# tuffy/libdvd-audio

Measured on AMD Instinct MI355X. Metric: decoded PCM Msamples/s (bit-exact) on 6ch/96k/24b MLP, higher is better.
Workload: dtype int32 (int64 accumulate)

## Files before the change

libdvd-audio_amd/csrc/mlp_decode.h:

```cpp
#pragma once
#include <hip/hip_runtime.h>
#if defined(__HIP_DEVICE_COMPILE__) && !defined(__gfx950__)
#error "mlp_decode.h is written for gfx950 (MI355X): hand-placed s_waitcnt encodings and gfx950 inline asm"
#endif
#include <stdint.h>
#include <type_traits>
#include "mlp_bounds.h"
#include "mlp_index.h"
#include "mlp_tables.h"

namespace mlp {

constexpr int DEC_THREADS = 128;
constexpr int DEC_WAVES = DEC_THREADS / 64;
constexpr int MAXCH = 8;
constexpr int MAXMAT = 6;
constexpr int RING_PLANES = 8;
constexpr int RING_DWORDS = RING_PLANES * 4;
constexpr int CHUNK_DWORDS = 16;
constexpr int OUT_ROWS = 4;
constexpr uint32_t YIELD_LONELY = 48;
#ifndef DVDA_HDR_GATE_TURNS
#define DVDA_HDR_GATE_TURNS 32
#endif
// ... 133 lines not shown
    uint32_t total_lanes;
    unsigned long long *dbg;
    int32_t *fir_ws;
    int32_t *fb;
    const int32_t *init_fir;
    DecodeSummary *summary;
    uint32_t interleaved;
    uint32_t wav_bits;
    uint32_t coop_min_seg;
    const uint32_t *hetero;
    const uint32_t *lane_seg;
    const uint32_t *cls;
    uint32_t only_S;
    uint32_t *seg_meta;
    uint32_t *yield_req;
    const uint32_t *seg_check;
    const uint32_t *list;
    uint32_t list_base, list_n;
    const uint32_t *list_n_ptr;
    const uint4 *plan;
    int32_t *res;
    uint32_t *brec;
    uint32_t *frec;
    WsCaps caps;
    uint32_t coop;
    struct CoopState *coop_state;
    struct CoopResult *coop_result;
    uint32_t coop_fresh;
};

constexpr uint32_t COOP_MAX_SEG = 4096;
constexpr uint32_t COOP_MAX_AU = 32768;
__device__ __forceinline__ bool coop_takes(const DecodeArgs &a)
{
    if (a.coop)
        return a.coop == 64u;
    uint32_t n_seg = *a.n_seg_ptr;
    if (n_seg > a.max_seg)
        n_seg = a.max_seg;
    return n_seg <= COOP_MAX_SEG && a.seg_fbase[n_seg] <= COOP_MAX_AU;
}



__device__ __forceinline__ int32_t mask_q(int32_t x, uint32_t q)
{
    return (int32_t)((uint32_t)x & (0xFFFFFFFFu << q));
}
__device__ __forceinline__ uint32_t nib(uint32_t pack, uint32_t i) { return (pack >> (4 * i)) & 0xFu; }
__device__ __forceinline__ int32_t lo16(uint32_t v) { return (int32_t)(v << 16) >> 16; }
__device__ __forceinline__ int32_t hi16(uint32_t v) { return (int32_t)v >> 16; }

__device__ __forceinline__ int32_t huff_center(uint32_t codebook, uint32_t lb)
{
    if (codebook) {
        const int ss = (int)lb + 2 - (int)codebook;
        return 7 * (1 << lb) + (ss >= 0 ? (1 << ss) : 0);
    }
    const int ss = (int)lb - 1;
    return ss >= 0 ? (1 << ss) : 0;
}

__device__ __forceinline__ uint32_t be32(uint32_t v) { return __builtin_bswap32(v); }
template <int RD = RING_DWORDS>
__device__ __forceinline__ void ring_store16(uint32_t *dst, const uint4 &a, const uint4 &b, const uint4 &c,
                                             const uint4 &d, bool first_plane)
{
    const uint32_t a0 = be32(a.x);
    uint32_t *const e = dst - 15 * 64;
    if (first_plane)
        dst[-RD * 64] = a0;
    e[15 * 64] = a0;         e[14 * 64] = be32(a.y); e[13 * 64] = be32(a.z); e[12 * 64] = be32(a.w);
    e[11 * 64] = be32(b.x);  e[10 * 64] = be32(b.y); e[9 * 64] = be32(b.z);  e[8 * 64] = be32(b.w);
    e[7 * 64] = be32(c.x);   e[6 * 64] = be32(c.y);  e[5 * 64] = be32(c.z);  e[4 * 64] = be32(c.w);
    e[3 * 64] = be32(d.x);   e[2 * 64] = be32(d.y);  e[1 * 64] = be32(d.z);  e[0 * 64] = be32(d.w);
}

template <int RD>
__device__ __forceinline__ void ring_store4(uint32_t *dst, const uint4 &a, bool first_plane)
{
    const uint32_t a0 = be32(a.x);
    if (first_plane)
        dst[-RD * 64] = a0;
    dst[0] = a0;
    dst[-1 * 64] = be32(a.y);
    dst[-2 * 64] = be32(a.z);
    dst[-3 * 64] = be32(a.w);
}

__device__ __forceinline__ void ring_fill_sync(const uint4 *src, uint32_t *dst, bool first_plane)
{
    const uint4 a = src[0], b = src[1], c = src[2], d = src[3];
    ring_store16(dst, a, b, c, d, first_plane);
}

__device__ __attribute__((noinline)) int64_t iir_mac(const int32_t *ws, uint32_t stride)
{
    int64_t acc = 0;
    for (uint32_t j = 0; j < 8; j++)
        acc += (int64_t)ws[(size_t)j * stride] * (int64_t)ws[(size_t)(8 + j) * stride];
    return acc;
}

__device__ __attribute__((noinline)) void iir_push(int32_t *ws, uint32_t stride, int32_t v)
{
    for (int j = 7; j > 0; j--)
        ws[(size_t)(8 + j) * stride] = ws[(size_t)(8 + j - 1) * stride];
    ws[(size_t)8 * stride] = v;
}

template <int RD, int G>
struct BitReaderT {
    const uint4 *gsrc;
    uint32_t *ring;
    uint32_t max_chunk;
    uint32_t pos;
    uint32_t fillpos;
    uint32_t lo_valid;

    __device__ __forceinline__ uint32_t *slot(uint32_t d) const
    {
        return ring + ((RD - (d & (RD - 1))) << 6);
    }
    __device__ __forceinline__ uint64_t window() const
    {
        const uint32_t *p = ring + ((~(pos >> 5) & (RD - 1)) << 6);
        return ((uint64_t)p[64] << 32) | p[0];
    }
    __device__ __forceinline__ uint32_t window_lds() const
    {
        return (uint32_t)(uintptr_t)ring + ((~(pos >> 5) & (RD - 1)) << 8);
    }
    __device__ __forceinline__ int32_t ahead() const
    {
        return (int32_t)((fillpos << 5) - (pos & ~31u)) >> 5;
    }
    __device__ __forceinline__ void filled()
    {
        fillpos += G;
        if (fillpos - lo_valid > (uint32_t)RD)
            lo_valid = fillpos - RD;
    }
    __device__ __forceinline__ uint32_t fill_src() const
    {
        const uint32_t last = max_chunk + (uint32_t)(CHUNK_DWORDS - G);
        return fillpos < last ? fillpos : last;
    }
    __device__ __forceinline__ bool room() const { return ahead() <= (int32_t)(RD - G); }
    __device__ __forceinline__ void fill_sync()
    {
        if constexpr (G == CHUNK_DWORDS) {
            ring_fill_sync(gsrc + (fill_src() >> 2), slot(fillpos), (fillpos & (RD - 1)) == 0);
            filled();
        } else {
            uint4 q[4];
            const int32_t n = fill_issue(q);
            fill_commit(q, n);
        }
    }
    template <int MAXG = 4>
    __device__ __forceinline__ int32_t fill_issue(uint4 (&q)[MAXG]) const
    {
        static_assert(G == CHUNK_DWORDS || (G == 4 && RD == 16), "the small ring is 16 dwords filled by 16-byte granules");
        int32_t n = room() ? (RD - ahead()) >> 2 : 0;
        if (MAXG < 4 && n > MAXG)
            n = MAXG;
#pragma unroll
        for (int g = 0; g < MAXG; g++)
            if (g < n) {
                const uint32_t f = fillpos + 4u * g, last = max_chunk + (uint32_t)(CHUNK_DWORDS - G);
                q[g] = gsrc[(f < last ? f : last) >> 2];
            }
        return n;
    }
    template <int MAXG = 4>
    __device__ __forceinline__ void fill_commit(const uint4 (&q)[MAXG], int32_t n)
    {
#pragma unroll
        for (int g = 0; g < MAXG; g++)
            if (g < n) {
                ring_store4<RD>(slot(fillpos), q[g], (fillpos & (RD - 1)) == 0);
                filled();
            }
    }
    __device__ __forceinline__ void ensure(uint32_t n)
    {
#if defined(DVDA_EXP_STAMP)
        const unsigned long long t0_ = clock64();
        bool any_ = false;
#endif
        while (__builtin_expect(__any(ahead() < (int32_t)n), 0)) {
            if (room())
                fill_sync();
#if defined(DVDA_EXP_STAMP)
            any_ = true;
#endif
        }
#if defined(DVDA_EXP_STAMP)
        if (any_) {
            fill_cyc += clock64() - t0_;
            fill_n++;
        }
#endif
    }
#if defined(DVDA_EXP_STAMP)
    unsigned long long fill_cyc = 0, fill_n = 0;
#endif
    __device__ __forceinline__ void seek_byte(uint64_t byte_pos)
    {
        const uint32_t t = (uint32_t)(byte_pos >> 2);
        if (!((int32_t)(t - lo_valid) >= 0 && (int32_t)(fillpos - t) > 0)) {
            fillpos = t & ~(uint32_t)(G - 1);
            lo_valid = fillpos;
        }
        pos = (uint32_t)byte_pos << 3;
    }
    __device__ __forceinline__ uint64_t tell_near(uint64_t ref_bits) const
    {
        return ref_bits + (uint64_t)(int64_t)(int32_t)(pos - (uint32_t)ref_bits);
    }
    __device__ __forceinline__ bool past(uint32_t end_bits_lo) const { return (int32_t)(pos - end_bits_lo) > 0; }
    __device__ __forceinline__ uint32_t peek32()
    {
        ensure(2);
        return (uint32_t)((window() << (pos & 31u)) >> 32);
    }
    __device__ __forceinline__ uint32_t read(uint32_t n)
    {
        const uint32_t top = peek32();
        pos += n;
        return n ? top >> (32 - n) : 0u;
    }
    __device__ __forceinline__ uint32_t read_resident(uint32_t n)
    {
        const uint32_t top = (uint32_t)((window() << (pos & 31u)) >> 32);
        pos += n;
        return (top >> 1) >> (31u - n);
    }
    __device__ __forceinline__ int32_t read_signed_resident(uint32_t n)
    {
        const uint32_t top = (uint32_t)((window() << (pos & 31u)) >> 32);
        pos += n;
        return n ? (int32_t)top >> ((32u - n) & 31u) : 0;
    }
    __device__ __forceinline__ int32_t read_signed(uint32_t n)
    {
        if (n == 0)
            return 0;
        const int32_t v = (int32_t)peek32() >> (32 - n);
        pos += n;
        return v;
    }
};

using BitReader = BitReaderT<RING_DWORDS, CHUNK_DWORDS>;
constexpr int DUO_RING = 16, DUO_GRAN = 4;

__host__ __device__ constexpr uint32_t hot_word(uint32_t cb, uint32_t lb, uint32_t q, uint32_t shift)
{
    return lb | (q << 5) | ((shift + q) << 10) |
           (cb ? ((7u - (8u >> cb)) << 16) | ((cb == 1 ? 9u : cb == 2 ? 7u : 6u) << 20) | ((4u - cb) << 24) |
                 ((28u + cb) << 26) | (1u << 31)
               : 0u);
}
__device__ __forceinline__ uint32_t hot_cb(uint32_t hw) { return (hw >> 26) & 3u; }
__device__ __forceinline__ uint32_t hot_lb(uint32_t hw) { return hw & 31u; }
__device__ __forceinline__ uint32_t hot_q(uint32_t hw) { return (hw >> 5) & 15u; }
__host__ __device__ constexpr uint32_t cold_word(uint32_t iir_order, uint32_t fir_order, uint32_t fir_shift, uint32_t iir_shift)
{
    return iir_order | (fir_order << 4) | (fir_shift << 8) | (iir_shift << 12);
}

__device__ __forceinline__ uint32_t huff_decode_top(uint32_t top, uint32_t hw)
{
    const uint32_t a = (top >> ((hw >> 26) & 31u)) + ((hw >> 16) & 0x307u);
    const uint32_t n = (uint32_t)__clz((int)((top & 0x3F800000u) | 0x00400000u));
    const uint32_t up = ((hw >> 20) & 0x10Fu) + n, dn = 0x108u - n;
    uint32_t d = 0x40000000u - (top & 0x7F800000u);
    asm("" : "+v"(d));
    uint32_t ms = (uint32_t)((int32_t)d >> 31);
    asm("" : "+v"(ms));
    uint32_t val = (up & ms) | (dn & ~ms);
    asm("" : "+v"(val));
    const uint32_t e = (n << 8) + val;
    uint32_t m = (uint32_t)((int32_t)top >> 31);
    asm("" : "+v"(m));
    return ((a & m) | (e & ~m)) & (uint32_t)((int32_t)hw >> 31);
}

__device__ __forceinline__ uint32_t huff_decode(uint32_t cb, uint32_t t)
{
    return huff_decode_top(t << 23, hot_word(cb, 0u, 0u, 0u));
}

struct SubPark {
    uint32_t flags, block_size, min_ch, max_ch, max_mat_ch, noise_shift, seed, matrix_len, bypass_mask, outch_pack,
             oshift_pack, qss_pack, nslots, iir_any, ss_end_bit, rows_left, blocks_in_frame, chk, gl, seg_lane;
    bool have_restart, seg_iir;
    uint32_t *brec, *brec_end, *brec_base;
};

template <int NS, bool PAIRED, bool GENERAL, bool ILV = false, bool PARSE = false, bool DUO = false, bool WAVO = false>
__global__ __launch_bounds__(DEC_THREADS, 2) void k_decode(DecodeArgs a)
{
    static_assert(!(GENERAL && PARSE), "one mode at a time");
    static_assert(!DUO || (!PAIRED && !GENERAL && NS == 6), "the two-substream lane is a one-lane fast-pass / parse instance");
    static_assert(GENERAL == PAIRED, "lane pairs are the sequential pass's layout, and its only one");
    constexpr uint32_t L = PAIRED ? 2u : 1u;
    if (!GENERAL && a.only_S && a.cls[a.only_S - 1u] == 0)
        return;
    if (!GENERAL && !PARSE && coop_takes(a))
        return;
    constexpr int THREADS = DEC_THREADS;
    constexpr int WAVES = THREADS / 64;
    constexpr int TP = 6;
    constexpr int RD = DUO ? DUO_RING : RING_DWORDS;
    constexpr int RG = DUO ? DUO_GRAN : CHUNK_DWORDS;
    using Reader = BitReaderT<RD, RG>;
    __shared__ uint32_t s_ring[WAVES][DUO ? 2 : 1][RD + 1][64];
    __shared__ int32_t s_out[GENERAL ? 1 : WAVES][TP][OUT_ROWS][GENERAL ? 1 : 64];
    constexpr bool XCH = PAIRED;
    __shared__ int32_t s_xch[XCH ? WAVES : 1][MAXCH][XCH ? 64 : 1];
    __shared__ uint32_t s_nchained[WAVES];
    __shared__ uint16_t s_cold[WAVES][NS][64];

    if (threadIdx.x < WAVES)
        s_nchained[threadIdx.x] = 0;
    __syncthreads();

    const int lane = threadIdx.x & 63;
    const int wv = threadIdx.x >> 6;
    const uint32_t wg_id = blockIdx.x;
    const uint32_t gl0 = wg_id * THREADS + threadIdx.x;
    uint32_t n_seg = *a.n_seg_ptr;
    if (n_seg > a.max_seg)
        n_seg = a.max_seg;
    const uint32_t item = gl0 / L;
    uint32_t segi = item;
    bool active = segi < n_seg;
    if (!GENERAL && !PARSE && active && *a.hetero)
        segi = DVDA_AT(a.lane_seg, item, a.caps.max_seg, BT_LANE_SEG);
    if (!GENERAL && !PARSE && segi >= n_seg) {
        active = false;
        segi = n_seg;
    }
    if (GENERAL || PARSE) {
        active = item < a.list_n && (a.list_n_ptr == nullptr || item < *a.list_n_ptr) && (!PARSE || item < DVDA_AT(a.plan, n_seg, a.caps.max_seg + 1u, BT_PLAN).y);
        segi = 0;
        if (active) {
            const uint32_t e = DVDA_AT(a.list, a.list_base + item, GENERAL ? a.caps.max_streams : a.caps.max_seg, BT_LIST);
            segi = GENERAL ? DVDA_AT(a.streams, e, a.caps.max_streams, BT_STREAMS).first_seg : e;
            active = segi < n_seg;
        }
        if (!active)
            segi = n_seg;
    }

    SegRec sr;
    sr.off = sr.end = 0;
    sr.stream = 0;
    sr.nframes = 0;
    sr.flags = 0;
    sr.sync = 0;
    sr.ndrop = 0;
    sr.prev = 0xFFFFFFFFu;
    uint32_t fbase = 0, stream_sync = 0, stream_first = 0;
    if (active) {
        sr = DVDA_AT(a.seg, segi, a.caps.max_seg, BT_SEG);
        stream_first = DVDA_AT(a.streams, sr.stream, a.caps.max_streams, BT_STREAMS).first_seg;
        if (stream_first == 0xFFFFFFFFu) {
            active = false;
            stream_first = segi;
        } else {
            stream_sync = a.streams[sr.stream].sync;
            fbase = a.seg_fbase[segi] - DVDA_AT(a.seg_fbase, stream_first, a.caps.max_seg + 1u, BT_FBASE);
        }
    }
    const uint32_t S = (stream_sync >> 24) & 0xF;
    const uint32_t sub = DUO ? 1u : gl0 - item * L;
    uint32_t gl = segi * 2u + sub;
    uint32_t seg_lane = gl;
    const uint32_t assignment = (stream_sync >> 16) & 0x1F;
    const uint32_t rpa = rows_per_au((stream_sync >> 8) & 0xF);
    const uint32_t nch_out = channel_count(assignment);
    const uint32_t wavepk = wave_pack(assignment);
    const uint32_t wave_inv = ILV ? wave_inv_pack(assignment) : 0u;
    uint32_t status = 0;
    if (active && (sr.flags & ST_FATAL_INDEX))
        active = false;
    if (active && (sub >= S || sr.nframes == 0))
        active = false;
    bool mine = GENERAL || !a.only_S || S == a.only_S;
    if (!mine)
        active = false;
    if (active && S > (DUO ? 2u : L)) {
        status |= ST_ENVELOPE;
        active = false;
    }
    if (DUO && S != 2u)
        active = false;
    if (active && (rpa == 0 || nch_out == 0)) {
        status |= ST_ENVELOPE;
        active = false;
    }
    const bool is_last_sub = (sub + 1 == S);
    const bool owner = is_last_sub;

    uint64_t out_base = 0, out_stride = 0;
    if (active && !PARSE) {
        out_base = a.out_off[sr.stream];
        out_stride = a.out_stride[sr.stream];
    }
    uint64_t row0 = (uint64_t)fbase * rpa;
    uint64_t row_limit = row0 + (uint64_t)(sr.nframes - sr.ndrop) * rpa;
    constexpr bool seq = GENERAL;
    bool resume_from_init = false;
    int32_t *fbuf = nullptr;
    if (GENERAL && active) {
        const uint32_t st_j = a.seg_status[segi];
        if (st_j & ST_CHAINED) {
            if (a.init_fir)
                resume_from_init = true;
            else {
                status |= ST_ENVELOPE;
                active = false;
            }
        }
        fbuf = a.fb + (size_t)item * FB_WORDS;
        if (active && !DVDA_RANGE_OK((size_t)item * FB_WORDS, FB_WORDS, a.caps.fb, BT_FB)) {
            status |= ST_CAPACITY;
            active = false;
        }
        if (active) {
            atomicAnd(&a.seg_status[segi], ST_DEFERRED | ST_FATAL_INDEX | ST_TRUNCATED | ST_SYNC_CHANGE);
            row0 = 0;
            row_limit = ~0ull;
        }
    }
    uint32_t seg_R = 0;
    uint32_t *brec = nullptr, *brec_end = nullptr, *brec_base = nullptr;
    uint32_t *frec = nullptr;
    if (PARSE && active) {
        const uint4 pl = DVDA_AT(a.plan, segi, a.caps.max_seg + 1u, BT_PLAN);
        const uint32_t st_j = a.seg_status[segi];
        seg_R = (sr.nframes - sr.ndrop) * rpa;
        out_base = (uint64_t)pl.x * 8u;
        out_stride = seg_R;
        row0 = 0;
        row_limit = seg_R;
        const uint32_t cap = brec_capacity(seg_R);
        brec = a.brec + brec_offset(pl.x, pl.y, sub, seg_R);
        brec_base = brec;
        brec_end = brec + cap;
        frec = a.frec + (uint64_t)(pl.x / 40u) * FREC_WORDS;
        (void)st_j;
        atomicAnd(&a.seg_status[segi], ST_DEFERRED | ST_FATAL_INDEX | ST_TRUNCATED | ST_SYNC_CHANGE);
        if (!DVDA_RANGE_OK(out_base, 8ull * seg_R, a.caps.res, BT_RES) ||
            !DVDA_RANGE_OK(brec_offset(pl.x, pl.y, sub, seg_R), cap, a.caps.brec, BT_BREC) ||
            !DVDA_RANGE_OK((uint64_t)(pl.x / 40u) * FREC_WORDS, (uint64_t)(sr.nframes - sr.ndrop) * FREC_WORDS, a.caps.frec, BT_FREC)) {
            status |= ST_CAPACITY;
            active = false;
        }
    }
    if (active && !DVDA_RANGE_OK(gl, 1, a.caps.lanes, BT_META)) {
        status |= ST_CAPACITY;
        active = false;
    }
    uint32_t room = 0;
    {
        const uint64_t edge = out_stride < row_limit ? out_stride : row_limit;
// ... 723 lines not shown
                                    }
                                    if (fir_order && frames_done == 0 && blocks_in_frame == 0)
                                        status |= ST_CHAINED;
                                    const int32_t nsho = hoff - huff_center(codebook, lb);
                                    const uint32_t npk = hot_word(codebook, lb, q, shift);
                                    if (kr < (uint32_t)NS)
                                        *cold = (uint16_t)cold_word(iir_order, fir_order, fir_shift, iir_shift);
#pragma unroll
                                    for (int kk = 0; kk < NS; kk++)
                                        if ((uint32_t)kk == kr) {
                                            pk[kk] = npk;
                                            sho[kk] = nsho;
                                            if (new_fir) {
#pragma unroll
                                                for (int j = 0; j < 4; j++) {
                                                    if constexpr (!CFU) {
                                                        cf[kk][CFU ? 0 : j] = (int32_t)ncf[j];
                                                    } else {
                                                        cf[kk][CFU ? 2 * j : 0] = lo16(ncf[j]);
                                                        cf[kk][CFU ? 2 * j + 1 : 0] = hi16(ncf[j]);
                                                    }
                                                }
                                            }
                                        }
                                    iir_any = (iir_any & ~(1u << k)) | ((iir_order ? 1u : 0u) << k);
                                    if (PARSE) {
                                        const bool with_iir = new_iir && iir_order != 0;
                                        if (brec + 2 * BREC_STRIDE + (with_iir ? BREC_IIR_WORDS : 0) > brec_end) {
                                            seq_needed = true;
                                        } else {
                                            uint32_t *w = brec + BREC_SLOT * k;
                                            w[2] = shift | (q << 4) | (fir_order << 8) | (iir_order << 12) |
                                                   (new_iir ? 1u << 16 : 0u);
#pragma unroll
                                            for (int j = 0; j < 4; j++)
                                                w[3 + j] = new_fir ? ncf[j] : cf_old[j];
                                            w[7] = 0;
                                            chg_mask |= 1u << k;
                                            if (with_iir) {
                                                const int32_t *ws = a.iir_ws + (size_t)(k * 16) * a.total_lanes + gl;
                                                brec_end -= BREC_IIR_WORDS;
                                                uint32_t *x = brec_end;
                                                for (uint32_t j = 0; j < 4; j++)
                                                    x[j] = ((uint32_t)ws[(size_t)(2 * j) * a.total_lanes] & 0xFFFFu) |
                                                           ((uint32_t)ws[(size_t)(2 * j + 1) * a.total_lanes] << 16);
                                                for (uint32_t j = 0; j < 8; j++)
                                                    x[4 + j] = (uint32_t)ws[(size_t)(8 + j) * a.total_lanes];
                                                w[7] = (uint32_t)(x - brec_base);
                                            }
                                        }
                                    }
                                }
                            }
                        }
                    }
                }
                DVDA_HSTAMP(3);
                if (!have_restart && ok) {
                    ok = false;
                    err = no_restart_yet();
                }
                hdr_parsed = true;
                if (PARSE && iir_any)
                    seg_iir = true;
                if (PARSE && ok && chg_mask) {
#pragma unroll
                    for (int kk = 0; kk < 6; kk++) {
                        brec[BREC_SLOT * kk] = rows_done;
                        brec[BREC_SLOT * kk + 1] = (chg_mask >> kk) & 1u;
                    }
                    brec += BREC_STRIDE;
                }
                if (PARSE && ok && (seq_needed || (hdr_restart && blocks_in_frame))) {
                    status |= ST_SEQ;
                    active = false;
                }
                if (mat_mine) {
                    qss_A = qss_pack;
                    mmc_A = max_mat_ch;
                }
                const uint32_t cold_ml = matrix_len;
                if (matrix_class_change)
                    status |= ST_MIDFRAME;
                if (!ok) {
                    status |= err;
                    active = false;
                } else if (PARSE && !active) {
                } else if (!GENERAL && !PARSE && (iir_any != 0 || cold_ml > 2)) {
                    status |= ST_COLD;
                    active = false;
                } else if (!GENERAL && !PARSE && (status & ST_CHAINED)) {
                    active = false;
                    if (!(DUO && probe))
                        atomicAdd(&s_nchained[wv], 1u);
                    if (sr.prev != 0xFFFFFFFFu)
                        __hip_atomic_store(&DVDA_AT(a.yield_req, sr.prev, a.caps.max_seg, BT_YIELD), 1u, __ATOMIC_RELAXED, __HIP_MEMORY_SCOPE_AGENT);
                } else {
                    rows_left = block_size;
                    blocks_in_frame++;
                    if (!GENERAL && !PARSE && frames_done < 2 &&
                        __hip_atomic_load(&s_nchained[wv], __ATOMIC_RELAXED, __HIP_MEMORY_SCOPE_WORKGROUP) >= YIELD_LONELY) {
                        status |= ST_YIELD;
                        active = false;
                    }
                }
            }
                if constexpr (DUO) {
                    if (pass == 0u && me)
                        swap_sub();
                    if (!PARSE && pass == 0u && me && !active && first0 && !(status & ~ST_INFO)) {
                        probe = true;
                        active = true;
                    }
                    if (pass == 1u && probe)
                        active = false;
                }
            }
            if constexpr (DUO) {
                if (active && have_restart && P0.have_restart && (P0.min_ch != 0u || min_ch != P0.max_ch + 1u)) {
                    status |= PARSE ? ST_SEQ : ST_COLD;
                    active = false;
                }
            }
        }
        if (hdr_now) {
            DVDA_HSTAMP(4);
#if defined(DVDA_EXP_STAMP)
            hstamp_acc[5] += rd.fill_cyc + (DUO ? rx.fill_cyc : 0ull);
            hfills += rd.fill_n + (DUO ? rx.fill_n : 0ull);
            hcount++;
#endif
        }
        if (!__any(active))
            break;
        DVDA_STAMP(0);

        if (active) {
            if constexpr (DUO) {
                while (__builtin_expect(__any(rd.ahead() < 8 || rx.ahead() < 8), 0)) {
                    DVDA_COV(14);
                    uint4 q[1];
                    const int32_t n0 = rx.template fill_issue<1>(q);
                    rx.template fill_commit<1>(q, n0);
                    const int32_t n1 = rd.template fill_issue<1>(q);
                    rd.template fill_commit<1>(q, n1);
                }
            } else {
            if (rd.ahead() < 12)
                DVDA_COV(14);
            rd.ensure(12);
            }
        }
        DVDA_STAMP(7);
        const bool pf = active && rd.room();
        const bool pfx = DUO && active && rx.room();
        uint4 p0, p1, p2, p3;
        asm volatile("" : "=v"(p0.x), "=v"(p0.y), "=v"(p0.z), "=v"(p0.w), "=v"(p1.x), "=v"(p1.y), "=v"(p1.z), "=v"(p1.w),
                          "=v"(p2.x), "=v"(p2.y), "=v"(p2.z), "=v"(p2.w), "=v"(p3.x), "=v"(p3.y), "=v"(p3.z), "=v"(p3.w));
        bool flush = false;
        const uint32_t frames_before = frames_done;
        uint64_t flush_row = 0;
        if constexpr (DUO) {
            if (pfx)
                p0 = rx.gsrc[rx.fill_src() >> 2];
            if (pf)
                p1 = rd.gsrc[rd.fill_src() >> 2];
        } else {
        if (pf) {
            const uint32_t c = rd.fillpos < rd.max_chunk ? rd.fillpos : rd.max_chunk;
            const uint4 *src = rd.gsrc + (c >> 2);
            p0 = src[0];
            p1 = src[1];
            p2 = src[2];
            p3 = src[3];
        }
        }
        DVDA_STAMP(1);

        uint32_t bypass_bits = 0;
        int32_t val[NS];
        auto row_head_any = [&]() {
            if (__any(bypass_mask != 0)) {
                const uint32_t cnt = (uint32_t)__popc(bypass_mask);
                const uint32_t field = rd.read_resident(cnt);
                const uint32_t b0 = bypass_mask & 1u, b1 = (bypass_mask >> 1) & 1u;
                bypass_bits = (b0 & (field >> ((cnt - 1u) & 31u))) | ((b1 & (field >> ((cnt - 1u - b0) & 31u))) << 1);
                if ((GENERAL || PARSE) && __builtin_expect(__any((bypass_mask >> 2) != 0), 0)) {
                    if (bypass_mask >> 2)
                        DVDA_COV(10);
                    uint32_t rank = b0 + b1;
#pragma unroll
                    for (int m = 2; m < MAXMAT; m++) {
                        const uint32_t bit = (bypass_mask >> m) & 1u;
                        bypass_bits |= (bit & (field >> ((cnt - 1u - rank) & 31u))) << m;
                        rank += bit;
                    }
                }
            }
            if constexpr (DUO)
                rx.pos += (uint32_t)__popc(P0.bypass_mask);
            uint32_t cpos = DUO ? rx.pos : rd.pos;
            uint32_t cbase = (uint32_t)(uintptr_t)(DUO ? rx.ring : rd.ring) + (uint32_t)((RD - 1) << 8);
            auto cur_window_lds = [&]() -> uint32_t { return cbase - ((cpos << 3) & (uint32_t)((RD - 1) << 8)); };
            uint64_t win = DUO ? rx.window() : rd.window();
            const uint32_t n_sub0 = DUO ? P0.max_ch + 1u : 0u;
            uint32_t msb_or = 0;
            const bool wave_iir = GENERAL && __any(iir_any != 0);
#pragma unroll
            for (int k = 0; k < NS; k++) {
                const bool in = DUO ? (uint32_t)k <= max_ch : (uint32_t)k < nslots;
                if (k > 0)
                    asm volatile("s_waitcnt lgkmcnt(0)" : "+v"(win));
                if constexpr (DUO) {
                    if (k > 0) {
                        const bool sw = (uint32_t)k == n_sub0;
                        if (__any(sw)) {
                            if (sw) {
                                rx.pos = cpos;
                                cpos = rd.pos;
                                cbase = (uint32_t)(uintptr_t)rd.ring + (uint32_t)((RD - 1) << 8);
                                win = rd.window();
                            }
                        }
                    }
                }
                val[k] = 0;
                if (k >= 2 && !__any(in))
                    continue;
                if (in) {
                const uint32_t hw = pk[k];
                const uint32_t lb = hw & 31u;
                const uint32_t ofs = cpos & 31u;
                const uint32_t top = (uint32_t)((win << ofs) >> 32);
                const uint32_t e = huff_decode_top(top, hw);
                const uint32_t msb = e & 0xFFu;
                const uint32_t len = e >> 8;
                msb_or |= msb;
                const uint32_t o2 = ofs + len;
                cpos += len + lb;
                const uint32_t top2 = (uint32_t)((win << o2) >> 32);
                const uint32_t lsbv = (top2 >> 1) >> (~hw & 31u);
                if (k + 1 < NS)
                    asm volatile("ds_read2st64_b32 %0, %2 offset1:1" : "+v"(win), "+v"(sp[k][0]) : "v"(cur_window_lds()));
                uint32_t ml = (msb << (hw & 31u)) + lsbv;
                asm("" : "+v"(ml));
                const uint32_t resq = ml + (uint32_t)sho[k];
                const uint32_t q5 = (hw >> 5) & 31u;
                int32_t value;
                if constexpr (PARSE) {
                    value = (int32_t)(resq << q5);
                    (void)wave_iir;
                } else {
                auto tap = [&](int j) -> int32_t {
                    if constexpr (CFU)
                        return cf[k][CFU ? j : 0];
                    else
                        return (j & 1) ? hi16((uint32_t)cf[k][CFU ? 0 : j >> 1]) : lo16((uint32_t)cf[k][CFU ? 0 : j >> 1]);
                };
                int64_t acc0 = (int64_t)tap(0) * (int64_t)st_get(k, 0);
                int64_t acc1 = (int64_t)tap(1) * (int64_t)st_get(k, 1);
                acc0 += (int64_t)tap(2) * (int64_t)st_get(k, 2);
                acc1 += (int64_t)tap(3) * (int64_t)st_get(k, 3);
                acc0 += (int64_t)tap(4) * (int64_t)st_get(k, 4);
                acc1 += (int64_t)tap(5) * (int64_t)st_get(k, 5);
                acc0 += (int64_t)tap(6) * (int64_t)st_get(k, 6);
                acc1 += (int64_t)tap(7) * (int64_t)st_get(k, 7);
                int64_t acc = acc0 + acc1;
                bool iir_on = false;
                if (__builtin_expect(wave_iir, 0)) {
                    iir_on = in && ((iir_any >> k) & 1u);
                    if (iir_on)
                        DVDA_COV(11);
                    if (iir_on)
                        acc += iir_mac(a.iir_ws + (size_t)(k * 16) * a.total_lanes + gl, a.total_lanes);
                }
                value = (int32_t)(((uint32_t)(acc >> ((hw >> 10) & 63u)) + resq) << q5);
                {
                    uint32_t vhi;
                    asm("" : "=v"(vhi));
                    const uint64_t vpair = (uint64_t)(uint32_t)value | ((uint64_t)vhi << 32);
                    asm("v_pk_mov_b32 %0, %1, %0 op_sel:[1,0]" : "+v"(sp[k][3]) : "v"(sp[k][2]));
                    asm("v_pk_mov_b32 %0, %1, %0 op_sel:[1,0]" : "+v"(sp[k][2]) : "v"(sp[k][1]));
                    asm("v_pk_mov_b32 %0, %1, %0 op_sel:[1,0]" : "+v"(sp[k][1]) : "v"(sp[k][0]));
                    asm("v_pk_mov_b32 %0, %1, %0 op_sel:[0,0]" : "+v"(sp[k][0]) : "v"(vpair));
                }
                if (__builtin_expect(wave_iir, 0)) {
                    if (iir_on) {
                        const int32_t ssum = (int32_t)(acc >> (((hw >> 10) & 63u) - hot_q(hw)));
                        iir_push(a.iir_ws + (size_t)(k * 16) * a.total_lanes + gl, a.total_lanes,
                                 (int32_t)((uint32_t)value - (uint32_t)ssum));
                    }
                }
                }
                val[k] = value;
                }
            }
            rd.pos = cpos;
            if (__builtin_expect((msb_or & 0x80u) != 0, 0)) {
                status |= ST_HUFFMAN;
                active = false;
            }
            DVDA_STAMP(2);
        };
        auto row_tail = [&](int32_t (&ch)[MAXCH]) {
            if (owner) {
                if (GENERAL) {
                    if (frame_rows >= (uint32_t)FB_ROWS) {
                        status |= ST_ENVELOPE;
                        active = false;
                    } else {
                        int32_t *fr = fbuf + (size_t)frame_rows * (MAXCH + 1);
#pragma unroll
                        for (int c = 0; c < MAXCH; c++)
                            fr[c] = ch[c];
                        fr[MAXCH] = (int32_t)bypass_bits;
                    }
                } else {
                    if constexpr (PARSE) {
#pragma unroll
// ... 85 lines not shown
                            uint32_t *F = frec + (size_t)au_idx * FREC_WORDS;
                            if (!DVDA_RANGE_OK((size_t)(F - a.frec), FREC_WORDS, a.caps.frec, BT_FREC))
                                F = a.frec;
                            F[0] = noise_shift | (matrix_len << 8) | (max_mat_ch << 16);
                            F[1] = outch_pack;
                            F[2] = qss_pack;
                            F[3] = oshift_pack;
#pragma unroll
                            for (int m = 0; m < 2; m++) {
#pragma unroll
                                for (int j = 0; j < 4; j++)
                                    F[4 + m * 5 + j] = mreg[m][j];
                                F[4 + m * 5 + 4] = mnoise[m];
                            }
                            for (uint32_t m = 2; m < matrix_len; m++)
                                for (uint32_t j = 0; j < 5; j++)
                                    F[4 + m * 5 + j] = a.mat_ws[(size_t)(m * 5 + j) * a.total_lanes + gl];
                        }
                        au_idx++;
                        in_frame = false;
                        frames_done++;
                    }
                }
            } else
            if (__builtin_expect(active && rows_left == 0, 0)) {
                if (rd.read(1)) {
                    if (frame_rows != rpa && !seq) {
                        status |= ST_TIMING;
                        active = false;
                    }
                    if (rd.past(ss_end_bit)) {
                        status |= ST_EOF;
                        active = false;
                    }
                    if (active && (chk >> 2) == frames_done) {
                        status |= (chk & 1u) ? ST_PARITY : ST_CRC;
                        active = false;
                    }
                    if (PARSE && is_last_sub && active) {
                        uint32_t *F = frec + (size_t)au_idx * FREC_WORDS;
                        if (!DVDA_RANGE_OK((size_t)(F - a.frec), FREC_WORDS, a.caps.frec, BT_FREC))
                            F = a.frec;
                        F[0] = noise_shift | (matrix_len << 8) | (max_mat_ch << 16);
                        F[1] = outch_pack;
                        F[2] = qss_pack;
                        F[3] = oshift_pack;
#pragma unroll
                        for (int m = 0; m < 2; m++) {
#pragma unroll
                            for (int j = 0; j < 4; j++)
                                F[4 + m * 5 + j] = mreg[m][j];
                            F[4 + m * 5 + 4] = mnoise[m];
                        }
                        for (uint32_t m = 2; m < matrix_len; m++)
                            for (uint32_t j = 0; j < 5; j++)
                                F[4 + m * 5 + j] = a.mat_ws[(size_t)(m * 5 + j) * a.total_lanes + gl];
                    }
                    au_idx++;
                    if (GENERAL && is_last_sub && active) {
                        const uint64_t frow0 = row - frame_rows;
                        for (uint32_t r = 0; r < frame_rows; r++) {
                            const int32_t *fr = fbuf + (size_t)r * (MAXCH + 1);
                            int32_t ch[MAXCH];
#pragma unroll
                            for (int c = 0; c < MAXCH; c++)
                                ch[c] = fr[c];
                            rematrix(ch, (uint32_t)fr[MAXCH]);
                            const uint64_t orow = frow0 + r;
                            if (orow >= out_stride) {
                                status |= ST_OVERFLOW;
                            } else {
                                if (a.wav_bits) {
                                    const uint32_t nb = a.wav_bits >> 3;
                                    uint8_t *wb = reinterpret_cast<uint8_t *>(a.pcm + out_base) + orow * nch_out * nb;
                                    for (uint32_t c = 0; c < nch_out && c < 6u; c++) {
                                        int32_t v = 0;
#pragma unroll
                                        for (int cc = 0; cc < 6; cc++)
                                            if ((uint32_t)cc == c)
                                                v = ch[cc];
                                        const uint32_t u = wav_signed(v, a.wav_bits);
                                        for (uint32_t b = 0; b < nb; b++)
                                            wb[nib(wavepk, c) * nb + b] = (uint8_t)(u >> (8 * b));
                                    }
                                } else {
#pragma unroll
                                for (int c = 0; c < 6; c++)
                                    if ((uint32_t)c < nch_out)
                                        a.pcm[out_base + (a.interleaved ? orow * nch_out + nib(wavepk, c)
                                                                        : (uint64_t)nib(wavepk, c) * out_stride + orow)] = ch[c];
                                }
                            }
                            rows_written++;
                        }
                    }
                    in_frame = false;
                    frames_done++;
                } else if (rd.past(ss_end_bit)) {
                    status |= ST_EOF;
                    active = false;
                }
            }
        };
        int32_t ch[MAXCH];
        const bool in_row = active && (!HDR_GATE || (rows_left != 0 && (!DUO || P0.rows_left != 0)));
        if (in_row) {
            row_head_any();
            if (PAIRED) {
                const int slot0 = lane & ~1;
                int32_t(*X)[XCH ? 64 : 1] = s_xch[XCH ? wv : 0];
#pragma unroll
                for (int k = 0; k < NS; k++)
                    if ((uint32_t)k < nslots && min_ch + k < MAXCH)
                        X[min_ch + k][XCH ? slot0 : 0] = val[k];
                __builtin_amdgcn_fence(__ATOMIC_RELEASE, "wavefront");
                __builtin_amdgcn_wave_barrier();
                __builtin_amdgcn_fence(__ATOMIC_ACQUIRE, "wavefront");
#pragma unroll
                for (int c = 0; c < MAXCH; c++)
                    ch[c] = X[c][XCH ? slot0 : 0];
            } else {
#pragma unroll
                for (int c = 0; c < MAXCH; c++)
                    ch[c] = c < NS ? val[c < NS ? c : 0] : 0;
            }
            row_tail(ch);
        }
        if constexpr (GENERAL) {
            const int ended = frames_done != frames_before ? 1 : 0;
            const int other = __shfl_xor(ended, 1, 64);
            if (S == 2u && active && ended != other) {
                status |= ST_ENVELOPE;
                active = false;
            }
        }
        DVDA_STAMP(3);

#if defined(DVDA_EXP_STAMP)
        {
            asm volatile("s_waitcnt vmcnt(0)" ::: "memory");
            DVDA_STAMP(6);
        }
#endif
        __builtin_amdgcn_s_waitcnt(0x0F70);
        if constexpr (DUO) {
            if (pfx) {
                ring_store4<RD>(rx.slot(rx.fillpos), p0, (rx.fillpos & (RD - 1)) == 0);
                rx.filled();
            }
            if (pf) {
                ring_store4<RD>(rd.slot(rd.fillpos), p1, (rd.fillpos & (RD - 1)) == 0);
                rd.filled();
            }
        } else {
        if (pf) {
            ring_store16(rd.slot(rd.fillpos), p0, p1, p2, p3, (rd.fillpos & (RING_DWORDS - 1)) == 0);
            rd.filled();
        }
        }
        bool coop_out = false;
        if constexpr (ILV && !GENERAL && !PARSE) {
            if (!WAVO && ilv_direct && a.wav_bits == 0u && a.coop_min_seg && n_seg >= a.coop_min_seg)
                coop_out = __ballot(flush) == ~0ull;
        }
        if (coop_out) {
            const uint64_t doff = out_base + flush_row * 6u;
            const bool off32 = !__any((doff >> 32) != 0);
            const uint32_t d_lo = (uint32_t)doff, d_hi = (uint32_t)(doff >> 32);
            const int32_t *const T0 = &s_out[GENERAL ? 0 : wv][0][0][0];
            const uint32_t l6 = ((uint32_t)lane * 43691u) >> 18;
            const uint32_t pc = (uint32_t)lane - l6 * 6u;
            const int32_t *const Tl6 = T0 + pc * (4 * 64) + l6;
            const bool l60 = lane < 60;
#pragma unroll
            for (uint32_t it7 = 0; it7 < 7u; it7++) {
                const uint32_t o = l6 + 10u * it7;
                const uint32_t b_lo = (uint32_t)__shfl((int)d_lo, (int)o, 64);
                uint64_t eo = b_lo;
                if (!off32)
                    eo |= (uint64_t)(uint32_t)__shfl((int)d_hi, (int)o, 64) << 32;
                if (l60 && (it7 < 6u || o < 64u)) {
                    int32_t *const od = a.pcm + eo + pc * 4u;
                    const int32_t *const Tp = Tl6 + 10u * it7;
                    DVDA_STORE_V4_COOP(od, Tp[0], Tp[64], Tp[128], Tp[192]);
                }
            }
        }
        if (!GENERAL && !PARSE && ILV && flush && !coop_out) {
            const int32_t *Tl = &s_out[GENERAL ? 0 : wv][0][0][GENERAL ? 0 : lane];
            int32_t *dst = a.pcm + out_base + flush_row * nch_out;
            constexpr bool WAV_ELSEWHERE = !PAIRED && !WAVO && !DUO;
            if (WAVO || (!WAV_ELSEWHERE && __builtin_expect(a.wav_bits != 0, 0))) {
                const uint32_t nb = a.wav_bits >> 3;
                uint32_t *wd = reinterpret_cast<uint32_t *>(a.pcm + out_base) + (flush_row * nch_out * nb >> 2);
                if (ilv_direct && a.wav_bits == 24u) {
                    uint32_t d[18];
#pragma unroll
                    for (int g = 0; g < 6; g++) {
                        const int32_t o[4] = {Tl[(4 * g) * 64], Tl[(4 * g + 1) * 64], Tl[(4 * g + 2) * 64], Tl[(4 * g + 3) * 64]};
                        uint32_t t[3];
                        wav_pack4(o, 24u, t);
                        d[3 * g] = t[0];
                        d[3 * g + 1] = t[1];
                        d[3 * g + 2] = t[2];
                    }
#pragma unroll
                    for (int v = 0; v < 4; v++)
                        DVDA_STORE_V4_AT(wd, 16 * v, (int)d[4 * v], (int)d[4 * v + 1], (int)d[4 * v + 2], (int)d[4 * v + 3]);
                    DVDA_STORE_V2_AT(wd, 64, d[16], d[17]);
                } else {
                    uint32_t fi = 0, fw = 0;
                    for (uint32_t v = 0; v < nch_out; v++) {
                        int32_t o[4];
#pragma unroll
                        for (int j = 0; j < 4; j++) {
                            o[j] = ilv_direct ? Tl[(4 * v + j) * 64] : Tl[(nib(wave_inv, fw) * OUT_ROWS + fi) * 64];
                            fw++;
                            if (fw == nch_out) {
                                fw = 0;
                                fi++;
                            }
                        }
                        uint32_t d[3];
                        wav_pack4(o, a.wav_bits, d);
                        wd[nb * v] = d[0];
                        wd[nb * v + 1] = d[1];
                        if (nb == 3u)
                            wd[nb * v + 2] = d[2];
                    }
                }
            } else if (__builtin_expect(ilv_direct, 1)) {
#pragma unroll
                for (int v = 0; v < (OUT_ROWS * 6) / 4; v++)
                    DVDA_STORE_V4_AT(dst, 16 * v, Tl[(4 * v) * 64], Tl[(4 * v + 1) * 64], Tl[(4 * v + 2) * 64],
                                     Tl[(4 * v + 3) * 64]);
            } else if (__all(nch_out == 2u && vec_ok)) {
                const int32_t *c0 = Tl + nib(wave_inv, 0) * (OUT_ROWS * 64), *c1 = Tl + nib(wave_inv, 1) * (OUT_ROWS * 64);
                DVDA_STORE_V4_AT(dst, 0, c0[0], c1[0], c0[64], c1[64]);
                DVDA_STORE_V4_AT(dst, 16, c0[128], c1[128], c0[192], c1[192]);
            } else {
                uint32_t fi = 0, fw = 0;
                for (uint32_t v = 0; v < (uint32_t)OUT_ROWS * 6u / 4u; v++) {
                    if (v * 4u < (uint32_t)OUT_ROWS * nch_out) {
                        int32_t o[4];
#pragma unroll
                        for (int j = 0; j < 4; j++) {
                            o[j] = Tl[(nib(wave_inv, fw) * OUT_ROWS + fi) * 64];
                            fw++;
                            if (fw == nch_out) {
                                fw = 0;
                                fi++;
                            }
                        }
                        if (vec_ok) {
                            DVDA_STORE_V4(dst + 4 * v, o[0], o[1], o[2], o[3]);
                        } else {
#pragma unroll
                            for (int j = 0; j < 4; j++)
                                dst[4 * v + j] = o[j];
                            DVDA_COV(13);
                        }
                    }
                }
            }
        }
        bool coop_flush = false;
        if constexpr (PARSE && !GENERAL)
            coop_flush = __ballot(flush) == ~0ull;
        if (PARSE && flush) {
            int32_t(*T)[OUT_ROWS][GENERAL ? 1 : 64] = s_out[GENERAL ? 0 : wv];
            int32_t *dst = a.res + out_base + (flush_row >> 2) * 32u;
            if (!DVDA_RANGE_OK(out_base + (flush_row >> 2) * 32u, 32, a.caps.res, BT_RES))
                dst = a.res;
            if (!coop_flush) {
#pragma unroll
            for (int c = 0; c < TP; c++)
                DVDA_STORE_V4_AT(dst, 16 * c, T[c][0][GENERAL ? 0 : lane], T[c][1][GENERAL ? 0 : lane],
                                 T[c][2][GENERAL ? 0 : lane], T[c][3][GENERAL ? 0 : lane]);
            }
            DVDA_STORE_V4_AT(dst, 16 * 6, pq_s[0], pq_s[1], pq_s[2], pq_s[3]);
        }
        if constexpr (PARSE && !GENERAL) {
            if (coop_flush) {
                const int32_t *dsrc = a.res + out_base + (flush_row >> 2) * 32u;
                if (!flush || !DVDA_RANGE_OK(out_base + (flush_row >> 2) * 32u, 32, a.caps.res, BT_RES))
                    dsrc = a.res;
                const uint32_t d_lo = (uint32_t)(uintptr_t)dsrc, d_hi = (uint32_t)((uintptr_t)dsrc >> 32);
                const int32_t *const T0 = &s_out[wv][0][0][0];
                for (uint32_t it6 = 0; it6 < 6u; it6++) {
                    const uint32_t q = it6 * 64u + (uint32_t)lane;
                    const uint32_t o = (q * 43691u) >> 18;
                    const uint32_t pc = q - o * 6u;
                    const uint32_t b_lo = (uint32_t)__shfl((int)d_lo, (int)o, 64), b_hi = (uint32_t)__shfl((int)d_hi, (int)o, 64);
                    int32_t *const od = reinterpret_cast<int32_t *>(((uint64_t)b_hi << 32) | b_lo) + pc * 4u;
                    const int32_t *const Tp = T0 + pc * (OUT_ROWS * 64) + o;
                    DVDA_STORE_V4_PAD(od, Tp[0], Tp[64], Tp[128], Tp[192]);
                }
            }
        }
        if (!GENERAL && !PARSE && !ILV && flush) {
            int32_t(*T)[OUT_ROWS][GENERAL ? 1 : 64] = s_out[GENERAL ? 0 : wv];
#pragma unroll
            for (int c = 0; c < 6; c++) {
                if ((uint32_t)c < nch_out) {
                    const uint32_t wc = nib(wavepk, c);
                    int32_t *dst = a.pcm + out_base + (uint64_t)wc * out_stride + flush_row;
// ... 200 lines not shown
```

Baseline: 253,000.

## Refill single-lane bitstream ring in 16-byte granules gated by wave-wide low-water mark

For the non-paired, non-DUO decode instances, the per-lane 32-dword bit ring is now refilled in 4-dword granules, up to four per turn. The prefetch is issued only when some lane in the wave has at most 16 dwords buffered, replacing the unconditional 16-dword chunk prefetch whenever the ring had room. The sync fill path also gains a granule variant for the 32-dword ring. The aim is fewer global loads and LDS stores per row and less register pressure on turns that need no refill. The cost is extra per-lane arithmetic, possibly more frequent partial refills, and a risk of stalls if the low-water threshold is too low.

Result: faster. 259,400, median of 6 (+2.6%).

```diff
diff --git a/libdvd-audio_amd/csrc/mlp_decode.h b/libdvd-audio_amd/csrc/mlp_decode.h
--- a/libdvd-audio_amd/csrc/mlp_decode.h
+++ b/libdvd-audio_amd/csrc/mlp_decode.h
@@ -309,6 +309,18 @@
         if constexpr (G == CHUNK_DWORDS) {
             ring_fill_sync(gsrc + (fill_src() >> 2), slot(fillpos), (fillpos & (RD - 1)) == 0);
             filled();
+        } else if constexpr (RD > 16) {
+            uint4 q[4];
+            const int32_t r = (RD - ahead()) >> 2;
+            const int32_t n = r < 4 ? r : 4;
+            const uint32_t end = max_chunk + (uint32_t)CHUNK_DWORDS;
+#pragma unroll
+            for (int g = 0; g < 4; g++) {
+                const uint32_t e = fillpos + 4u * g + 4u;
+                q[g] = gsrc[((e < end ? e : end) >> 2) - 1u];
+            }
+            __builtin_amdgcn_s_waitcnt(0x0F70);
+            fill_commit(q, n);
         } else {
             uint4 q[4];
             const int32_t n = fill_issue(q);
@@ -318,9 +330,10 @@
     template <int MAXG = 4>
     __device__ __forceinline__ int32_t fill_issue(uint4 (&q)[MAXG]) const
     {
-        static_assert(G == CHUNK_DWORDS || (G == 4 && RD == 16), "the small ring is 16 dwords filled by 16-byte granules");
+        static_assert(G == CHUNK_DWORDS || (G == 4 && (RD == 16 || RD == 32)),
+                      "granule fills: the two small rings of a two-substream lane, or the 32-dword ring");
         int32_t n = room() ? (RD - ahead()) >> 2 : 0;
-        if (MAXG < 4 && n > MAXG)
+        if ((MAXG < 4 || RD > 16) && n > MAXG)
             n = MAXG;
 #pragma unroll
         for (int g = 0; g < MAXG; g++)
@@ -472,7 +485,8 @@
     constexpr int WAVES = THREADS / 64;
     constexpr int TP = 6;
     constexpr int RD = DUO ? DUO_RING : RING_DWORDS;
-    constexpr int RG = DUO ? DUO_GRAN : CHUNK_DWORDS;
+    constexpr bool WAVE_FILL = !DUO && !PAIRED;
+    constexpr int RG = DUO ? DUO_GRAN : WAVE_FILL ? 4 : CHUNK_DWORDS;
     using Reader = BitReaderT<RD, RG>;
     __shared__ uint32_t s_ring[WAVES][DUO ? 2 : 1][RD + 1][64];
     __shared__ int32_t s_out[GENERAL ? 1 : WAVES][TP][OUT_ROWS][GENERAL ? 1 : 64];
@@ -1502,8 +1516,10 @@
             }
         }
         DVDA_STAMP(7);
-        const bool pf = active && rd.room();
+        constexpr int32_t FILL_TURN = 16;
+        const bool pf = !WAVE_FILL && active && rd.room();
         const bool pfx = DUO && active && rx.room();
+        int32_t fn = 0;
         uint4 p0, p1, p2, p3;
         asm volatile("" : "=v"(p0.x), "=v"(p0.y), "=v"(p0.z), "=v"(p0.w), "=v"(p1.x), "=v"(p1.y), "=v"(p1.z), "=v"(p1.w),
                           "=v"(p2.x), "=v"(p2.y), "=v"(p2.z), "=v"(p2.w), "=v"(p3.x), "=v"(p3.y), "=v"(p3.z), "=v"(p3.w));
@@ -1515,6 +1531,22 @@
                 p0 = rx.gsrc[rx.fill_src() >> 2];
             if (pf)
                 p1 = rd.gsrc[rd.fill_src() >> 2];
+        } else if constexpr (WAVE_FILL) {
+            if (__any(active && rd.ahead() <= FILL_TURN)) {
+                const int32_t r = (RD - rd.ahead()) >> 2;
+                fn = active ? (r < 4 ? r : 4) : 0;
+                const uint32_t end = rd.max_chunk + (uint32_t)CHUNK_DWORDS;
+                const uint32_t last = end - 4u * (uint32_t)fn;
+                const uint4 *src = rd.gsrc + ((rd.fillpos < last ? rd.fillpos : last) >> 2);
+                if (fn > 0)
+                    p0 = src[0];
+                if (fn > 1)
+                    p1 = src[1];
+                if (fn > 2)
+                    p2 = src[2];
+                if (fn > 3)
+                    p3 = src[3];
+            }
         } else {
         if (pf) {
             const uint32_t c = rd.fillpos < rd.max_chunk ? rd.fillpos : rd.max_chunk;
@@ -1906,6 +1938,24 @@
                 ring_store4<RD>(rd.slot(rd.fillpos), p1, (rd.fillpos & (RD - 1)) == 0);
                 rd.filled();
             }
+        } else if constexpr (WAVE_FILL) {
+            if (__any(fn > 0)) {
+                const uint32_t f = rd.fillpos;
+                if (fn > 0) {
+                    ring_store4<RD>(rd.slot(f), p0, (f & (RD - 1)) == 0);
+                    if (fn > 1) {
+                        ring_store4<RD>(rd.slot(f + 4u), p1, ((f + 4u) & (RD - 1)) == 0);
+                        if (fn > 2) {
+                            ring_store4<RD>(rd.slot(f + 8u), p2, ((f + 8u) & (RD - 1)) == 0);
+                            if (fn > 3)
+                                ring_store4<RD>(rd.slot(f + 12u), p3, ((f + 12u) & (RD - 1)) == 0);
+                        }
+                    }
+                    rd.fillpos = f + 4u * (uint32_t)fn;
+                    if (rd.fillpos - rd.lo_valid > (uint32_t)RD)
+                        rd.lo_valid = rd.fillpos - RD;
+                }
+            }
         } else {
         if (pf) {
             ring_store16(rd.slot(rd.fillpos), p0, p1, p2, p3, (rd.fillpos & (RING_DWORDS - 1)) == 0);
```
